# AuburnSounds/gamut

Measured on AMD Instinct MI355X. Metric: Mpixels/sec decoded (batched 1080p JPEG 4:2:0), higher is better.
Workload: dtype int32; 1 GPU; batch 1024 x 1920x1080 baseline JPEG 4:2:0, IDCT + freq-domain chroma upsample + YCbCr->RGBA8, coefficients + max_zag of the q 90 smooth-plus-noise generator; parity_check=not run (bench.py --full checks against the oracle before timing)

## Files before the change

gamut_amd/csrc/jpeg.hip:

```cpp
#include "common.hpp"
#include "jpeg_math.hpp"

namespace gamut {
namespace {

using namespace jpg;

constexpr int TILE_MCUS = 8;
#ifndef JPEG_H2V2_MCUS
#define JPEG_H2V2_MCUS 8
#endif
constexpr int H2V2_MCUS = JPEG_H2V2_MCUS;
constexpr int H2V2_THREADS = 32 * H2V2_MCUS;

struct JpegArgs {
    const int16_t* coeffs; int64_t coeff_stride;
    const uint8_t* max_zag; int64_t zag_stride;
    uint8_t* out; int64_t out_pitch; int64_t out_stride;
    int width, height;
    int mcus_per_row, mcus_per_col;
    int scan_type, out_comps;
    int count;
    const u32* tokens; const u32* strip_tab; const int64_t* tok_offs; const int64_t* strip_offs;
    int nt;
    int flip;
};

constexpr int BLK_STRIDE = 72;
constexpr int T1_INTS = 4 * H2V2_MCUS * BLK_STRIDE;
constexpr int H_INTS  = 2 * H2V2_MCUS * BLK_STRIDE;
constexpr int V_INTS  = 2 * H2V2_MCUS * BLK_STRIDE;
constexpr int LDS_INTS = T1_INTS + H_INTS + V_INTS;

__device__ __forceinline__ constexpr int phys_slot(int m) { constexpr int P[8] = { 0, 2, 1, 3, 6, 4, 7, 5 }; return P[m]; }

__device__ const u32 kMapPacked[2][4] __attribute__((aligned(16))) = {
    { pk16(E1a, E1b), pk16(E1c, E1d), pk16(E3a, E3b), pk16(E3c, E3d) }, { pk16(O0a, O0b), pk16(O0c, O0d), pk16(O2a, O2b), pk16(O2c, O2d) } };
__device__ const i32 kVTable[4][4] __attribute__((aligned(16))) = { { O0a, O0b, O0c, O0d }, { E1a, E1b, E1c, E1d }, { O2a, O2b, O2c, O2d }, { E3a, E3b, E3c, E3d } };
struct __attribute__((packed, aligned(1))) Dwords4u { u32 v[4]; };

__device__ __forceinline__ void wave_sync()
{
    __builtin_amdgcn_fence(__ATOMIC_RELEASE, "wavefront");
    __builtin_amdgcn_wave_barrier();
    __builtin_amdgcn_fence(__ATOMIC_ACQUIRE, "wavefront");
}
#ifndef JPEG_NT_LOADS
#define JPEG_NT_LOADS 1
#endif
__device__ __forceinline__ uint4 load_coeffs16(const int16_t* p)
{
    typedef u32 u32x4n __attribute__((ext_vector_type(4)));
    if (JPEG_NT_LOADS) { const u32x4n v = __builtin_nontemporal_load(reinterpret_cast<const u32x4n*>(p)); return make_uint4(v.x, v.y, v.z, v.w); }
    return *reinterpret_cast<const uint4*>(p);
}

__device__ __forceinline__ void store_px_nt(uint8_t* row_base, u32 voff, u32 px)
{
    asm volatile("global_store_dword %0, %1, %2 nt" :: "v"(voff), "v"(px), "s"(row_base));
}
__device__ __forceinline__ void store_px_plain(uint8_t* row_base, u32 voff, u32 px)
{
    asm volatile("global_store_dword %0, %1, %2" :: "v"(voff), "v"(px), "s"(row_base));
}

#ifndef JPEG_XCD_REMAP
#define JPEG_XCD_REMAP 1
#endif
#ifndef JPEG_STRIPS
#define JPEG_STRIPS 1
#endif
#ifndef JPEG_STRIPS_PACKED
#define JPEG_STRIPS_PACKED 5
#endif
#ifndef JPEG_UNROLL_STRIPS
#define JPEG_UNROLL_STRIPS 0
#endif
#ifndef JPEG_444_MCUS
#define JPEG_444_MCUS 10
#endif
#ifndef JPEG_444_MCUS_RGB8
#define JPEG_444_MCUS_RGB8 8
#endif
constexpr int plain_mcus(int scan_type, int oc = 4) { return scan_type == GAMUT_JPGD_GRAYSCALE ? 32 : scan_type == GAMUT_JPGD_YH1V1 ? (oc == 3 ? JPEG_444_MCUS_RGB8 : JPEG_444_MCUS) : 8; }
constexpr int plain_strips(int scan_type) { return (scan_type == GAMUT_JPGD_GRAYSCALE || scan_type == GAMUT_JPGD_YH1V1) ? 8 : 1; }
constexpr int plain_threads(int scan_type) { return scan_type == GAMUT_JPGD_YH1V1 ? ((JPEG_444_MCUS > JPEG_444_MCUS_RGB8 ? JPEG_444_MCUS : JPEG_444_MCUS_RGB8) * 3 * 8 + 63) / 64 * 64 : 256; }
#ifndef JPEG_ABLATE
#define JPEG_ABLATE 0
#endif

#ifndef JPEG_MIN_WAVES
#define JPEG_MIN_WAVES 0
#endif
template <int OC, bool TOK = false, bool NT = true>
#if JPEG_MIN_WAVES
__global__ __launch_bounds__(H2V2_THREADS, JPEG_MIN_WAVES) void k_jpeg_h2v2(JpegArgs a)
#else
__global__ __launch_bounds__(H2V2_THREADS) void k_jpeg_h2v2(JpegArgs a)
#endif
{
    __shared__ __attribute__((aligned(16))) i32 lds[LDS_INTS];
    i32* const T1 = lds;
    i32* const Hs = T1 + T1_INTS;
    i32* const Vs = Hs + H_INTS;
    i32* const T2 = T1;
    int16_t* const Xs = reinterpret_cast<int16_t*>(Vs);

    constexpr int STRIPS = OC == 4 ? JPEG_STRIPS : JPEG_STRIPS_PACKED;
    const int t = threadIdx.x;
#if JPEG_XCD_REMAP
    const int img = blockIdx.z * 8 + (blockIdx.x & 7), mcu_y = blockIdx.y, tile0 = (blockIdx.x >> 3) * STRIPS;
    if (img >= a.count) return;
#else
    const int img = blockIdx.z, mcu_y = blockIdx.y, tile0 = blockIdx.x * STRIPS;
#endif
    const int n_tiles = (a.mcus_per_row + H2V2_MCUS - 1) / H2V2_MCUS;
    const int16_t* cbase = TOK ? nullptr : a.coeffs + (int64_t)img * a.coeff_stride + ((int64_t)mcu_y * a.mcus_per_row + tile0 * H2V2_MCUS) * (6 * 64);
    uint8_t* obase = a.out + (int64_t)img * a.out_stride + (a.flip ? (int64_t)(a.height - 1 - (mcu_y * 16 + 15)) : (int64_t)(mcu_y * 16)) * a.out_pitch +
                     (int64_t)tile0 * (H2V2_MCUS * 16 * OC);
    const uint8_t* zbase = a.max_zag ? a.max_zag + (int64_t)img * a.zag_stride + ((int64_t)mcu_y * a.mcus_per_row + tile0 * H2V2_MCUS) * 6 : nullptr;

    const int b = t >> 3, r = t & 7, m = b >> 2, q = b & 3;
    const int cbk = t >> 4, k = (t >> 1) & 7, half = t & 1;
    const uint4 mp = *reinterpret_cast<const uint4*>(kMapPacked[half]);
    const int ci = (t >> 2) & 3, cj = t & 3;
    const int pe = ((ci & 1) << 1) | (ci >> 1);
    const int po = 4 + ((((ci & 1) ^ 1) << 1) | (ci >> 1));
    const int4 vc = *reinterpret_cast<const int4*>(kVTable[cj]);
    const i32 sg = (cj & 1) ? -1 : 1;

    const ColourConsts cc = colour_consts();
    const i32 c_round = col_round();
    const int lx = m * 16 + (q & 1) * 8 + r;
    const int ly0 = (q >> 1) * 8;
    const bool all_rows = a.height - mcu_y * 16 >= 16;
    const int rows_here = a.height - mcu_y * 16 - ly0;
    const u32 pitch = (u32)a.out_pitch;
    const u32 voff = (u32)(lx * 4) + (u32)(a.flip ? 8 - ly0 : ly0) * pitch;

    const u32 yoff = (u32)(m * 384 + q * 64 + r * 8), yoff0 = (u32)(q * 64 + r * 8);
    const u32 coff = (u32)((cbk >> 1) * 384 + 256 + (cbk & 1) * 64 + k * 8), coff0 = (u32)(256 + (cbk & 1) * 64 + k * 8);
    auto fetch = [&](int tile, uint4& yv, uint4& cv) {
        const int here = a.mcus_per_row - tile * H2V2_MCUS;
        const int16_t* base = cbase + (int64_t)(tile - tile0) * (H2V2_MCUS * 384);
#if JPEG_ABLATE == 3
        yv = make_uint4(t + tile, t * 3, t * 5, t * 7); cv = make_uint4(t * 11, t, t * 13, t * 17 + tile); (void)here; (void)base;
#else
        yv = load_coeffs16(base + (m < here ? yoff : yoff0));
        cv = load_coeffs16(base + ((cbk >> 1) < here ? coff : coff0));
#endif
    };
    auto fetch_zag = [&](int tile) -> u32 {
        if (!zbase) return 64u;
        const int here = a.mcus_per_row - tile * H2V2_MCUS;
        return m < here ? (u32)zbase[((tile - tile0) * H2V2_MCUS + m) * 6 + q] : 1u;
    };
    auto fetch_tokens = [&](int tile, uint4& yv, uint4& cv) {
        if constexpr (TOK) {
            uint8_t* const ctile = reinterpret_cast<uint8_t*>(Hs);
            __syncthreads();
            static_assert((H_INTS + V_INTS) * 4 >= 64 * 128, "the coefficient tile (any 6-bit block index) fits the H / V area");
            *reinterpret_cast<uint4*>(ctile + t * 16) = make_uint4(0, 0, 0, 0);
            *reinterpret_cast<uint2*>(ctile + H2V2_THREADS * 16 + t * 8) = make_uint2(0, 0);
            const u32* st = a.strip_tab + a.strip_offs[img] + ((int64_t)mcu_y * n_tiles + tile);
            const u32 t0 = st[0], t1 = st[1];
            const u32* tk = a.tokens + a.tok_offs[img];
            __syncthreads();
            for (u32 idx = t0 + (u32)t; idx < t1; idx += H2V2_THREADS) {
                const u32 w = tk[idx];
                *reinterpret_cast<uint16_t*>(ctile + ((w >> 26) << 7) + ((w >> 19) & 126u)) = (uint16_t)w;
            }
            __syncthreads();
            yv = *reinterpret_cast<const uint4*>(ctile + yoff * 2);
            cv = *reinterpret_cast<const uint4*>(ctile + coff * 2);
            __syncthreads();
        }
    };
    uint4 yrow, crow;
    u32 yzag = 64;
    if (!TOK && tile0 < n_tiles) { fetch(tile0, yrow, crow); yzag = fetch_zag(tile0); }

#if JPEG_UNROLL_STRIPS
    #pragma unroll
#else
    #pragma unroll 1
#endif
    for (int s = 0; s < STRIPS; ++s) {
        const int tile = tile0 + s;
        if (tile >= n_tiles) break;
        const int mcu_x0 = tile * H2V2_MCUS;
        const int mcus_here = min(H2V2_MCUS, a.mcus_per_row - mcu_x0);
        const bool mcu_live = m < mcus_here;
        uint8_t* const otile = obase + (size_t)s * (H2V2_MCUS * 16 * OC);
        if constexpr (TOK) { fetch_tokens(tile, yrow, crow); yzag = fetch_zag(tile); }
        uint4 ynext = yrow, cnext = crow;
        u32 znext = yzag;
        if (!TOK && s + 1 < STRIPS && tile + 1 < n_tiles) { fetch(tile + 1, ynext, cnext); znext = fetch_zag(tile + 1); }
        const bool y_sparse = zbase && __builtin_amdgcn_ballot_w64(yzag > 10u) == 0;

#if JPEG_ABLATE == 1
        if constexpr (OC == 4) {
            const u32 v0 = yrow.x ^ yrow.y ^ yrow.z ^ yrow.w ^ crow.x ^ crow.y ^ crow.z ^ crow.w;
            if (mcu_live && mcu_x0 * 16 + lx < a.width && all_rows) {
                #pragma unroll
                for (int i = 0; i < 8; ++i) store_px_nt(otile + (size_t)i * pitch, voff, v0 + i);
            }
            yrow = ynext; crow = cnext; yzag = znext; (void)y_sparse;
            continue;
        }
#endif

        if (y_sparse) {
            i32 tv[8];
            row_pass4_pairs(__builtin_amdgcn_perm(yrow.y, yrow.x, 0x05040100u), __builtin_amdgcn_perm(yrow.y, yrow.x, 0x07060302u), tv);
            if (r < 4) {
                i32* dst = T1 + b * BLK_STRIDE + r * 8;
                *reinterpret_cast<int4*>(dst)     = make_int4(tv[0], tv[1], tv[2], tv[3]);
                *reinterpret_cast<int4*>(dst + 4) = make_int4(tv[4], tv[5], tv[6], tv[7]);
            }
        } else {
            i32 tv[8];
            row_pass_packed(yrow, tv);
            i32* dst = T1 + b * BLK_STRIDE + r * 8;
            *reinterpret_cast<int4*>(dst)     = make_int4(tv[0], tv[1], tv[2], tv[3]);
            *reinterpret_cast<int4*>(dst + 4) = make_int4(tv[4], tv[5], tv[6], tv[7]);
        }
        {
            i32 hv[4];
            const u32 w0 = half ? crow.y : crow.x, w1 = half ? crow.w : crow.z;
            const u32 p13 = __builtin_amdgcn_perm(crow.y, crow.x, 0x07060302u), p57 = __builtin_amdgcn_perm(crow.w, crow.z, 0x07060302u);
            hv[0] = (i32)(short)(w0 & 0xFFFF);
            hv[1] = (i32)(short)(w1 & 0xFFFF);
            hv[2] = dot2(p13, mp.x, dot2(p57, mp.y, 512)) >> 10;
            hv[3] = dot2(p13, mp.z, dot2(p57, mp.w, 512)) >> 10;
            *reinterpret_cast<int4*>(Hs + cbk * BLK_STRIDE + k * 8 + half * 4) = make_int4(hv[0], hv[1], hv[2], hv[3]);
        }
        wave_sync();

        i32 ys[8];
        {
            const i32* src = T1 + b * BLK_STRIDE + r;
            i32 t0;
            if (y_sparse) {
                t0 = src[0];
                col_pass4_direct(t0, src[8], src[16], src[24], ys, c_round);
            } else {
                i32 tv[8];
                #pragma unroll
                for (int i = 0; i < 8; ++i) tv[i] = src[i * 8];
                col_pass<8>(tv, ys);
                t0 = tv[0];
            }
            if (zbase && __builtin_amdgcn_ballot_w64(yzag <= 2u) != 0) {
                const bool y_col1 = mcu_live && yzag <= 2u;
                const i32 v = col1_sample(t0);
                #pragma unroll
                for (int i = 0; i < 8; ++i) ys[i] = y_col1 ? v : ys[i];
            }
        }
        {
            const i32* he = Hs + cbk * BLK_STRIDE + pe;
            const i32* ho = Hs + cbk * BLK_STRIDE + po;
            const i32 pass_e = he[cj * 16], pass_o = ho[cj * 16];
            const i32 sum_e = mad24_1(vc.w, he[56], mad24_1(vc.z, he[40], mad24_1(vc.y, he[24], mad24_1(vc.x, he[8], 512)))) >> 10;
            const i32 sum_o = mad24_1(vc.w, ho[56], mad24_1(vc.z, ho[40], mad24_1(vc.y, ho[24], mad24_1(vc.x, ho[8], 512)))) >> 10;
            const i32 pa = wadd(pass_e, sum_e), pc = wadd(pass_o, sum_o);
            const i32 pu = wsub(pass_e, sum_e), pv = wsub(pass_o, sum_o);
            int16_t* dst = Xs + cbk * 64 + cj * 4 + pe;
            dst[0]  = (int16_t)wadd(pa, pc);
            dst[16] = (int16_t)wsub(pa, pc);
            dst[32] = (int16_t)mad24_1(wadd(pu, pv), sg, 0);
            dst[48] = (int16_t)mad24_1(wsub(pu, pv), sg, 0);
        }
        wave_sync();

        {
            const int mm = t >> 5, comp = (t >> 4) & 1, qq = (t >> 2) & 3, j = t & 3;
            const uint2 xp = *reinterpret_cast<const uint2*>(Xs + (mm * 2 + comp) * 64 + qq * 16 + j * 4);
            i32 tv[8];
            row_pass4_pairs(xp.x, xp.y, tv);
            i32* dst = T2 + (mm * 4 + qq) * BLK_STRIDE + (comp * 4 + j) * 8;
            *reinterpret_cast<int4*>(dst)     = make_int4(tv[0], tv[1], tv[2], tv[3]);
            *reinterpret_cast<int4*>(dst + 4) = make_int4(tv[4], tv[5], tv[6], tv[7]);
        }
        wave_sync();

        {
            i32 cbs[8], crs[8];
            const i32* src = T2 + b * BLK_STRIDE + r;
            col_pass4_direct(src[0], src[8], src[16], src[24], cbs, c_round);
            col_pass4_direct(src[32], src[40], src[48], src[56], crs, c_round);

            const bool px_live = mcu_live && mcu_x0 * 16 + lx < a.width;
            if constexpr (OC == 4) {
                auto store_px = [](uint8_t* row_base, u32 vo, u32 px) { if constexpr (NT) store_px_nt(row_base, vo, px); else store_px_plain(row_base, vo, px); };
                if (px_live) {
                    if (JPEG_ABLATE == 2) {
                        u32 acc = 0;
                        #pragma unroll
                        for (int i = 0; i < 8; ++i) acc += ycc_to_rgba(ys[i], cbs[i], crs[i], cc.kr, cc.kb, cc.kg);
                        if (acc == 0x12345679u) store_px_nt(otile, voff, acc);
                    } else
                    if (all_rows) {
                        #pragma unroll
                        for (int i = 0; i < 8; ++i) store_px(otile + (size_t)(a.flip ? 7 - i : i) * pitch, voff, ycc_to_rgba(ys[i], cbs[i], crs[i], cc.kr, cc.kb, cc.kg));
                    } else {
                        #pragma unroll
                        for (int i = 0; i < 8; ++i)
                            if (i < rows_here) store_px(otile + (size_t)(a.flip ? 7 - i : i) * pitch, voff, ycc_to_rgba(ys[i], cbs[i], crs[i], cc.kr, cc.kb, cc.kg));
                    }
                }
            } else {
                static_assert(OC == 3 || OC == 1, "output components");
                constexpr int BPR = 16 * H2V2_MCUS * OC;
                uint8_t* stage = reinterpret_cast<uint8_t*>(Hs);
                const int j = lx & 3;
                __syncthreads();
                #pragma unroll
                for (int i = 0; i < 8; ++i) {
                    const u32 px = ycc_to_rgba(ys[i], cbs[i], crs[i], cc.kr, cc.kb, cc.kg);
                    if constexpr (OC == 3) {
                        const u32 sel = j == 0 ? 0x04020100u : j == 1 ? 0x05040201u : 0x06050402u;
                        const u32 nx = (u32)__builtin_amdgcn_mov_dpp((int)px, 0xF9, 0xF, 0xF, true);
                        const u32 dw = __builtin_amdgcn_perm(nx, px, sel);
                        if (j < 3) *reinterpret_cast<u32*>(stage + (ly0 + i) * BPR + lx * 3 + j) = dw;
                    } else {
                        u32 v = rgb_to_luma(px) << (8 * j);
                        v |= (u32)__builtin_amdgcn_mov_dpp((int)v, 0xB1, 0xF, 0xF, true);
                        v |= (u32)__builtin_amdgcn_mov_dpp((int)v, 0x4E, 0xF, 0xF, true);
                        if (j == 0) *reinterpret_cast<u32*>(stage + (ly0 + i) * BPR + lx) = v;
                    }
                }
                __syncthreads();
                const int row_bytes = min(mcus_here * 16, a.width - mcu_x0 * 16) * OC;
                const int live_rows = min(16, a.height - mcu_y * 16);
                constexpr int CPR = BPR / 16;
                for (int c = t; c < 16 * CPR; c += H2V2_THREADS) {
                    const int row = c / CPR, off = (c - row * CPR) * 16;
                    if (row >= live_rows || off >= row_bytes) continue;
                    const uint4 v = *reinterpret_cast<const uint4*>(stage + row * BPR + off);
                    uint8_t* o = otile + (u32)(a.flip ? 15 - row : row) * pitch + (u32)off;
                    if (off + 16 <= row_bytes) {
                        if (a.nt) {
                            typedef u32 u32x4p __attribute__((ext_vector_type(4), aligned(4)));
                            __builtin_nontemporal_store(u32x4p{ v.x, v.y, v.z, v.w }, reinterpret_cast<u32x4p*>(o));
                        } else {
                            Dwords4u d; d.v[0] = v.x; d.v[1] = v.y; d.v[2] = v.z; d.v[3] = v.w;
                            *reinterpret_cast<Dwords4u*>(o) = d;
                        }
                    } else {
                        const u32 w[4] = { v.x, v.y, v.z, v.w };
                        for (int kk = 0; kk < row_bytes - off; ++kk) o[kk] = (uint8_t)(w[kk >> 2] >> ((kk & 3) * 8));
                    }
                }
                __syncthreads();
            }
        }
        wave_sync();
        yrow = ynext; crow = cnext; yzag = znext;
    }
}

struct __attribute__((packed, aligned(4))) Dwords4 { u32 v[4]; };
struct __attribute__((packed, aligned(1))) Dwords3 { u32 v[3]; };
struct __attribute__((packed, aligned(1))) Dword1 { u32 v; };

template <int ST, int OC, bool NT = true>
__global__ __launch_bounds__(plain_threads(ST)) void k_jpeg_plain(JpegArgs a)
{
    constexpr int NTHR = plain_threads(ST);
    static_assert(ST == GAMUT_JPGD_GRAYSCALE || ST == GAMUT_JPGD_YH1V1 || ST == GAMUT_JPGD_YH2V1 || ST == GAMUT_JPGD_YH1V2, "sampling mode");
    constexpr int BPM  = ST == GAMUT_JPGD_GRAYSCALE ? 1 : ST == GAMUT_JPGD_YH1V1 ? 3 : 4;
    constexpr int MH   = ST == GAMUT_JPGD_YH1V2 ? 16 : 8;
    constexpr int MCUS = plain_mcus(ST, OC);
    constexpr int NBLK = MCUS * BPM;
    static_assert(NBLK * 8 <= NTHR, "a thread per block row");
    constexpr int MW   = ST == GAMUT_JPGD_YH2V1 ? 16 : 8;
    constexpr int SW   = MCUS * MW;
    __shared__ __attribute__((aligned(16))) i32 T1[NBLK * BLK_STRIDE];
    __shared__ __attribute__((aligned(16))) uint8_t S[NBLK * 64];

    const int t = threadIdx.x;
    const int img = blockIdx.z * 8 + (blockIdx.x & 7), mcu_y = blockIdx.y, bx = blockIdx.x >> 3;
    if (img >= a.count) return;
    constexpr int PLAIN_STRIPS = plain_strips(ST);
    for (int strip = 0; strip < PLAIN_STRIPS; ++strip) {
    const int mcu_x0 = (bx * PLAIN_STRIPS + strip) * MCUS;
    if (mcu_x0 >= a.mcus_per_row) break;
    const int64_t blk0 = ((int64_t)mcu_y * a.mcus_per_row + mcu_x0) * BPM;
    const int16_t* cbase = a.coeffs + (int64_t)img * a.coeff_stride + blk0 * 64;
    const int mcus_here = min(MCUS, a.mcus_per_row - mcu_x0);
    const int b = t >> 3, r = t & 7;
    const bool blk_live = b < mcus_here * BPM;

    if (t < NBLK * 8) {
        uint4 row = make_uint4(0, 0, 0, 0);
        if (blk_live) row = load_coeffs16(cbase + (u32)(t * 8));
        i32 tv[8];
        row_pass_packed(row, tv);
        i32* dst = T1 + b * BLK_STRIDE + r * 8;
        *reinterpret_cast<int4*>(dst)     = make_int4(tv[0], tv[1], tv[2], tv[3]);
        *reinterpret_cast<int4*>(dst + 4) = make_int4(tv[4], tv[5], tv[6], tv[7]);
    }
    wave_sync();
    if (t < NBLK * 8) {
        i32 tv[8], sm[8];
        const i32* src = T1 + b * BLK_STRIDE + r;
        #pragma unroll
        for (int i = 0; i < 8; ++i) tv[i] = src[i * 8];
        col_pass<8>(tv, sm);
        if (a.max_zag) {
            bool col1 = false;
            if (blk_live) col1 = a.max_zag[(int64_t)img * a.zag_stride + blk0 + b] <= 2;
            const i32 v = col1_sample(tv[0]);
            #pragma unroll
            for (int i = 0; i < 8; ++i) sm[i] = col1 ? v : sm[i];
        }
        #pragma unroll
        for (int i = 0; i < 8; ++i) S[b * 64 + i * 8 + r] = (uint8_t)sm[i];
    }
    __syncthreads();

    uint8_t* obase = a.out + (int64_t)img * a.out_stride + (int64_t)(mcu_y * MH) * a.out_pitch + (int64_t)mcu_x0 * (MW * OC);
    const int rows_here = min(MH, a.height - mcu_y * MH);
    const int px_here = min(mcus_here * MW, a.width - mcu_x0 * MW);
    constexpr int GPR = SW / 4;
    for (int g = t; g < GPR * MH; g += NTHR) {
        const int y = g / GPR, x0 = (g - y * GPR) * 4;
        if (y >= rows_here || x0 >= px_here) continue;
        const int m = x0 / MW, xin = x0 - m * MW;
        u32 ys, px[4];
        if constexpr (ST == GAMUT_JPGD_GRAYSCALE) {
            ys = *reinterpret_cast<const u32*>(S + m * 64 + y * 8 + xin);
        } else if constexpr (ST == GAMUT_JPGD_YH1V1) {
            const uint8_t* sp = S + m * 192 + y * 8 + xin;
            ys = *reinterpret_cast<const u32*>(sp);
            const u32 cbs = *reinterpret_cast<const u32*>(sp + 64), crs = *reinterpret_cast<const u32*>(sp + 128);
            #pragma unroll
            for (int j = 0; j < 4; ++j) px[j] = ycc_to_rgba((ys >> (8 * j)) & 255, (cbs >> (8 * j)) & 255, (crs >> (8 * j)) & 255);
        } else if constexpr (ST == GAMUT_JPGD_YH1V2) {
            const uint8_t* mp = S + m * 256;
            ys = *reinterpret_cast<const u32*>(mp + (y >> 3) * 64 + (y & 7) * 8 + xin);
// ... 348 lines not shown
        i32 yv;
        if (st == GAMUT_JPGD_GRAYSCALE) {
            yv = s[ly * 8 + xin]; rgba = 0;
        } else if (st == GAMUT_JPGD_YH1V1) {
            const int o = ly * 8 + xin;
            yv = s[o]; rgba = ycc_to_rgba(yv, s[64 + o], s[128 + o]);
        } else if (st == GAMUT_JPGD_YH2V1) {
            yv = s[(xin >> 3) * 64 + ly * 8 + (xin & 7)];
            const int co = 2 * 64 + ly * 8 + (xin >> 1);
            rgba = ycc_to_rgba(yv, s[co], s[co + 64]);
        } else if (st == GAMUT_JPGD_YH1V2) {
            yv = s[(ly >> 3) * 64 + (ly & 7) * 8 + xin];
            const int co = 2 * 64 + (ly >> 1) * 8 + xin;
            rgba = ycc_to_rgba(yv, s[co], s[co + 64]);
        } else {
            const int o = ((ly >> 3) * 2 + (xin >> 3)) * 64 + (ly & 7) * 8 + (xin & 7);
            yv = s[o]; rgba = ycc_to_rgba(yv, s[4 * 64 + o], s[8 * 64 + o]);
        }
        uint8_t* o = obase + (int64_t)gy * a.out_pitch + (int64_t)gx * a.out_comps;
        if (st == GAMUT_JPGD_GRAYSCALE) {
            o[0] = (uint8_t)yv;
            if (a.out_comps >= 3) { o[1] = o[2] = (uint8_t)yv; if (a.out_comps == 4) o[3] = 255; }
        } else if (a.out_comps == 4) {
            o[0] = (uint8_t)rgba; o[1] = (uint8_t)(rgba >> 8); o[2] = (uint8_t)(rgba >> 16); o[3] = 255;
        } else if (a.out_comps == 3) {
            o[0] = (uint8_t)rgba; o[1] = (uint8_t)(rgba >> 8); o[2] = (uint8_t)(rgba >> 16);
        } else {
            o[0] = (uint8_t)rgb_to_luma(rgba);
        }
    }
}

}

int jpeg_reconstruct_launch(const int16_t* coeffs, int64_t coeff_stride,
                            const uint8_t* max_zag, int64_t zag_stride,
                            uint8_t* out, int64_t out_pitch, int64_t out_stride,
                            int width, int height, int scan_type, int out_comps,
                            int count, hipStream_t stream)
{
    if (width < 1 || height < 1 || width > 16384 || height > 16384)
        return set_error(GAMUT_HIP_ERR_INVALID_ARG, "jpeg_reconstruct: bad image size %dx%d", width, height);
    if (scan_type < GAMUT_JPGD_GRAYSCALE || scan_type > GAMUT_JPGD_YH2V2)
        return set_error(GAMUT_HIP_ERR_INVALID_ARG, "jpeg_reconstruct: bad scan type %d", scan_type);
    if (out_comps != 1 && out_comps != 3 && out_comps != 4)
        return set_error(GAMUT_HIP_ERR_INVALID_ARG, "jpeg_reconstruct: out_comps must be 1, 3 or 4");
    if (count < 0) return set_error(GAMUT_HIP_ERR_INVALID_ARG, "jpeg_reconstruct: negative count");
    if (count == 0) return GAMUT_HIP_OK;
    if (!coeffs || !out) return set_error(GAMUT_HIP_ERR_INVALID_ARG, "jpeg_reconstruct: null pointer");
    if (((uintptr_t)coeffs & 15) || (count > 1 && (coeff_stride & 7)))
        return set_error(GAMUT_HIP_ERR_INVALID_ARG, "jpeg_reconstruct: coefficient buffers must be 16-byte aligned");

    JpegArgs a{};
    a.coeffs = coeffs; a.coeff_stride = coeff_stride; a.max_zag = max_zag; a.zag_stride = zag_stride;
    a.out = out; a.out_pitch = out_pitch; a.out_stride = out_stride;
    a.width = width; a.height = height; a.scan_type = scan_type; a.out_comps = out_comps;
    const int mcu_w = (scan_type == GAMUT_JPGD_YH2V1 || scan_type == GAMUT_JPGD_YH2V2) ? 16 : 8;
    const int mcu_h = (scan_type == GAMUT_JPGD_YH1V2 || scan_type == GAMUT_JPGD_YH2V2) ? 16 : 8;
    a.mcus_per_row = (width + mcu_w - 1) / mcu_w;
    a.mcus_per_col = (height + mcu_h - 1) / mcu_h;
    const int tiles = (a.mcus_per_row + TILE_MCUS - 1) / TILE_MCUS;

    for (int i0 = 0; i0 < count; i0 += 65535) {
        const int n = count - i0 < 65535 ? count - i0 : 65535;
        JpegArgs c = a;
        c.count = n;
        c.coeffs += (int64_t)i0 * coeff_stride; c.out += (int64_t)i0 * out_stride;
        if (c.max_zag) c.max_zag += (int64_t)i0 * zag_stride;
        const dim3 grid(tiles, a.mcus_per_col, n);
        const int64_t apitch = out_pitch < 0 ? -out_pitch : out_pitch;
        const bool tuned = apitch > 0 && apitch < (1 << 27) &&
                           (out_comps != 4 || (((uintptr_t)out & 3) == 0 && (apitch & 3) == 0 && (out_stride & 3) == 0));
        if (tuned && out_pitch < 0 && scan_type == GAMUT_JPGD_YH2V2) { c.flip = 1; c.out_pitch = apitch; c.out += (int64_t)(height - 1) * out_pitch; }
        const bool on_lines = (((uintptr_t)out | (uintptr_t)apitch | (uintptr_t)(count > 1 ? (out_stride < 0 ? -out_stride : out_stride) : 0)) & 127u) == 0;
        c.nt = on_lines ? 1 : 0;
        const char* const cols_env = getenv("GAMUT_HIP_JPEG_COLS");
        const bool cols_tuned = !(cols_env && !strcmp(cols_env, "plain"));
        const int ps = plain_strips(scan_type);
        const int pm = plain_mcus(scan_type, out_comps);
        const dim3 grid32(8u * (unsigned)(((a.mcus_per_row + 31) / 32 + ps - 1) / ps), a.mcus_per_col, (n + 7) / 8);
        const dim3 grid_plain(8u * (unsigned)(((a.mcus_per_row + pm - 1) / pm + ps - 1) / ps), a.mcus_per_col, (n + 7) / 8);
        const int strips420 = out_comps == 4 ? JPEG_STRIPS : JPEG_STRIPS_PACKED;
        const unsigned groups420 = (unsigned)(((a.mcus_per_row + H2V2_MCUS - 1) / H2V2_MCUS + strips420 - 1) / strips420);
#if JPEG_XCD_REMAP
        const dim3 grid420(8u * groups420, a.mcus_per_col, (n + 7) / 8);
#else
        const dim3 grid420(groups420, a.mcus_per_col, n);
#endif
#define GAMUT_JPEG_PLAIN(ST, G) do { \
            if (out_comps == 4)      hipLaunchKernelGGL((k_jpeg_plain<ST, 4>), G, dim3(plain_threads(ST)), 0, stream, c);       \
            else if (out_comps == 3) { if (on_lines) hipLaunchKernelGGL((k_jpeg_plain<ST, 3>), G, dim3(plain_threads(ST)), 0, stream, c); else hipLaunchKernelGGL((k_jpeg_plain<ST, 3, false>), G, dim3(plain_threads(ST)), 0, stream, c); } \
            else                     { if (on_lines) hipLaunchKernelGGL((k_jpeg_plain<ST, 1>), G, dim3(plain_threads(ST)), 0, stream, c); else hipLaunchKernelGGL((k_jpeg_plain<ST, 1, false>), G, dim3(plain_threads(ST)), 0, stream, c); } } while (0)
        if (!tuned)                                   hipLaunchKernelGGL(k_jpeg_generic, grid, dim3(256), 0, stream, c);
        else if (scan_type == GAMUT_JPGD_GRAYSCALE)   GAMUT_JPEG_PLAIN(GAMUT_JPGD_GRAYSCALE, grid32);
        else if ((scan_type == GAMUT_JPGD_YH1V1 || scan_type == GAMUT_JPGD_GRAYSCALE) && cols_tuned) {
            const int waste32 = (32 - a.mcus_per_row % 32) % 32, waste24 = (24 - a.mcus_per_row % 24) % 24;
            const bool m24 = waste24 * 32 < waste32 * 24;
            const dim3 g(8u * (unsigned)(((a.mcus_per_row + (m24 ? 23 : 31)) / (m24 ? 24 : 32) + 1) / 2), a.mcus_per_col, (n + 7) / 8);
#define GAMUT_JPEG_COLS(ST, OC) do { if (m24) { if (on_lines) hipLaunchKernelGGL((k_jpeg_cols<ST, OC, 24>), g, dim3(192), 0, stream, c); else hipLaunchKernelGGL((k_jpeg_cols<ST, OC, 24, false>), g, dim3(192), 0, stream, c); } \
                                     else     { if (on_lines) hipLaunchKernelGGL((k_jpeg_cols<ST, OC, 32>), g, dim3(256), 0, stream, c); else hipLaunchKernelGGL((k_jpeg_cols<ST, OC, 32, false>), g, dim3(256), 0, stream, c); } } while (0)
            if (scan_type == GAMUT_JPGD_YH1V1) { if (out_comps == 4) GAMUT_JPEG_COLS(GAMUT_JPGD_YH1V1, 4); else if (out_comps == 3) GAMUT_JPEG_COLS(GAMUT_JPGD_YH1V1, 3); else GAMUT_JPEG_COLS(GAMUT_JPGD_YH1V1, 1); }
            else                               { if (out_comps == 4) GAMUT_JPEG_COLS(GAMUT_JPGD_GRAYSCALE, 4); else if (out_comps == 3) GAMUT_JPEG_COLS(GAMUT_JPGD_GRAYSCALE, 3); else GAMUT_JPEG_COLS(GAMUT_JPGD_GRAYSCALE, 1); }
#undef GAMUT_JPEG_COLS
        }
        else if (scan_type == GAMUT_JPGD_YH1V1)       GAMUT_JPEG_PLAIN(GAMUT_JPGD_YH1V1, grid_plain);
        else if ((scan_type == GAMUT_JPGD_YH2V1 || scan_type == GAMUT_JPGD_YH1V2) && cols_tuned) {
            const int waste32 = (32 - a.mcus_per_row % 32) % 32, waste24 = (24 - a.mcus_per_row % 24) % 24;
            const bool m24 = waste24 * 32 < waste32 * 24;
            const dim3 g(8u * (unsigned)(((a.mcus_per_row + (m24 ? 23 : 31)) / (m24 ? 24 : 32) + 1) / 2), a.mcus_per_col, (n + 7) / 8);
#define GAMUT_JPEG_COLS4(ST, OC) do { if (m24) { if (on_lines) hipLaunchKernelGGL((k_jpeg_cols4<ST, OC, 24>), g, dim3(192), 0, stream, c); else hipLaunchKernelGGL((k_jpeg_cols4<ST, OC, 24, false>), g, dim3(192), 0, stream, c); } \
                                      else     { if (on_lines) hipLaunchKernelGGL((k_jpeg_cols4<ST, OC, 32>), g, dim3(256), 0, stream, c); else hipLaunchKernelGGL((k_jpeg_cols4<ST, OC, 32, false>), g, dim3(256), 0, stream, c); } } while (0)
            if (scan_type == GAMUT_JPGD_YH2V1) { if (out_comps == 4) GAMUT_JPEG_COLS4(GAMUT_JPGD_YH2V1, 4); else if (out_comps == 3) GAMUT_JPEG_COLS4(GAMUT_JPGD_YH2V1, 3); else GAMUT_JPEG_COLS4(GAMUT_JPGD_YH2V1, 1); }
            else                               { if (out_comps == 4) GAMUT_JPEG_COLS4(GAMUT_JPGD_YH1V2, 4); else if (out_comps == 3) GAMUT_JPEG_COLS4(GAMUT_JPGD_YH1V2, 3); else GAMUT_JPEG_COLS4(GAMUT_JPGD_YH1V2, 1); }
#undef GAMUT_JPEG_COLS4
        }
        else if (scan_type == GAMUT_JPGD_YH2V1)       GAMUT_JPEG_PLAIN(GAMUT_JPGD_YH2V1, grid_plain);
        else if (scan_type == GAMUT_JPGD_YH1V2)       GAMUT_JPEG_PLAIN(GAMUT_JPGD_YH1V2, grid_plain);
        else if (out_comps == 4 && on_lines) hipLaunchKernelGGL(k_jpeg_h2v2<4>, grid420, dim3(H2V2_THREADS), 0, stream, c);
        else if (out_comps == 4) hipLaunchKernelGGL((k_jpeg_h2v2<4, false, false>), grid420, dim3(H2V2_THREADS), 0, stream, c);
        else if (out_comps == 3) hipLaunchKernelGGL(k_jpeg_h2v2<3>, grid420, dim3(H2V2_THREADS), 0, stream, c);
        else                     hipLaunchKernelGGL(k_jpeg_h2v2<1>, grid420, dim3(H2V2_THREADS), 0, stream, c);
#undef GAMUT_JPEG_PLAIN
        if (int rc = launch_status("jpeg_reconstruct")) return rc;
    }
    return GAMUT_HIP_OK;
}

int jpeg_reconstruct_tokens_launch(const uint32_t* tokens, const uint32_t* strip_tab, const int64_t* tok_offs, const int64_t* strip_offs,
                                   const uint8_t* max_zag, int64_t zag_stride, uint8_t* out, int64_t out_pitch, int64_t out_stride,
                                   int width, int height, int out_comps, int count, hipStream_t stream)
{
    if (width < 1 || height < 1 || width > 16384 || height > 16384 || count < 0 || (out_comps != 1 && out_comps != 3 && out_comps != 4) || !max_zag)
        return set_error(GAMUT_HIP_ERR_INVALID_ARG, "jpeg_reconstruct_tokens: bad arguments");
    if (count == 0) return GAMUT_HIP_OK;
    const int64_t apitch = out_pitch < 0 ? -out_pitch : out_pitch;
    if (apitch <= 0 || apitch >= (1 << 27) || (out_comps == 4 && ((((uintptr_t)out & 3) != 0) || (apitch & 3) || (out_stride & 3))))
        return set_error(GAMUT_HIP_ERR_INVALID_ARG, "jpeg_reconstruct_tokens: output rows must be dword-aligned for rgba8");
    JpegArgs a{};
    a.tokens = tokens; a.strip_tab = strip_tab; a.max_zag = max_zag; a.zag_stride = zag_stride;
    a.out = out; a.out_pitch = apitch; a.out_stride = out_stride;
    a.width = width; a.height = height; a.scan_type = GAMUT_JPGD_YH2V2; a.out_comps = out_comps;
    a.mcus_per_row = (width + 15) / 16; a.mcus_per_col = (height + 15) / 16;
    if (out_pitch < 0) { a.flip = 1; a.out += (int64_t)(height - 1) * out_pitch; }
    for (int i0 = 0; i0 < count; i0 += 65528) {
        const int n = count - i0 < 65528 ? count - i0 : 65528;
        JpegArgs c = a;
        c.count = n; c.out += (int64_t)i0 * out_stride; c.max_zag += (int64_t)i0 * zag_stride; c.tok_offs = tok_offs + i0; c.strip_offs = strip_offs + i0;
        const int strips420 = out_comps == 4 ? JPEG_STRIPS : JPEG_STRIPS_PACKED;
        const unsigned groups420 = (unsigned)(((a.mcus_per_row + H2V2_MCUS - 1) / H2V2_MCUS + strips420 - 1) / strips420);
#if JPEG_XCD_REMAP
        const dim3 grid420(8u * groups420, a.mcus_per_col, (n + 7) / 8);
#else
        const dim3 grid420(groups420, a.mcus_per_col, n);
#endif
        const bool on_lines = (((uintptr_t)out | (uintptr_t)apitch | (uintptr_t)(count > 1 ? (out_stride < 0 ? -out_stride : out_stride) : 0)) & 127u) == 0;
        c.nt = on_lines ? 1 : 0;
        if (out_comps == 4 && on_lines) hipLaunchKernelGGL((k_jpeg_h2v2<4, true>), grid420, dim3(H2V2_THREADS), 0, stream, c);
        else if (out_comps == 4) hipLaunchKernelGGL((k_jpeg_h2v2<4, true, false>), grid420, dim3(H2V2_THREADS), 0, stream, c);
        else if (out_comps == 3) hipLaunchKernelGGL((k_jpeg_h2v2<3, true>), grid420, dim3(H2V2_THREADS), 0, stream, c);
        else                     hipLaunchKernelGGL((k_jpeg_h2v2<1, true>), grid420, dim3(H2V2_THREADS), 0, stream, c);
        if (int rc = launch_status("jpeg_reconstruct_tokens")) return rc;
    }
    return GAMUT_HIP_OK;
}

}
```

Before: 813,900 Mpx/s.

## Split packed RGB/gray 4:2:0 path into its own software-pipelined kernel

Moves the OC==3/1 4:2:0 reconstruction into a separate kernel that uses buffer-resource loads, forces arguments into scalar registers, and overlaps the next strip's row pass with the current strip's staged store. It also adds a col-1 shortcut for very sparse Y blocks. The grid choice (XCD remap vs plain) becomes a runtime flag selected when the batch has fewer than 8 images. The benchmarked RGBA8 path only gains a PLAIN template variant and loses the OC branches, so it should be mostly unchanged for batch 1024.

```diff
diff --git a/gamut_amd/csrc/jpeg.hip b/gamut_amd/csrc/jpeg.hip
--- a/gamut_amd/csrc/jpeg.hip
+++ b/gamut_amd/csrc/jpeg.hip
@@ -21,6 +21,7 @@
     int mcus_per_row, mcus_per_col;
     int scan_type, out_comps;
     int count;
+    int plain_grid;
     const u32* tokens; const u32* strip_tab; const int64_t* tok_offs; const int64_t* strip_offs;
     int nt;
     int flip;
@@ -92,7 +93,7 @@
 #ifndef JPEG_MIN_WAVES
 #define JPEG_MIN_WAVES 0
 #endif
-template <int OC, bool TOK = false, bool NT = true>
+template <int OC, bool TOK = false, bool NT = true, bool PLAIN = false>
 #if JPEG_MIN_WAVES
 __global__ __launch_bounds__(H2V2_THREADS, JPEG_MIN_WAVES) void k_jpeg_h2v2(JpegArgs a)
 #else
@@ -106,14 +107,12 @@
     i32* const T2 = T1;
     int16_t* const Xs = reinterpret_cast<int16_t*>(Vs);
 
-    constexpr int STRIPS = OC == 4 ? JPEG_STRIPS : JPEG_STRIPS_PACKED;
+    static_assert(OC == 4, "rgba8");
+    constexpr int STRIPS = JPEG_STRIPS;
     const int t = threadIdx.x;
-#if JPEG_XCD_REMAP
-    const int img = blockIdx.z * 8 + (blockIdx.x & 7), mcu_y = blockIdx.y, tile0 = (blockIdx.x >> 3) * STRIPS;
+    const int img = PLAIN ? (int)blockIdx.z : (int)(blockIdx.z * 8 + (blockIdx.x & 7));
+    const int mcu_y = blockIdx.y, tile0 = (int)(PLAIN ? blockIdx.x : blockIdx.x >> 3) * STRIPS;
     if (img >= a.count) return;
-#else
-    const int img = blockIdx.z, mcu_y = blockIdx.y, tile0 = blockIdx.x * STRIPS;
-#endif
     const int n_tiles = (a.mcus_per_row + H2V2_MCUS - 1) / H2V2_MCUS;
     const int16_t* cbase = TOK ? nullptr : a.coeffs + (int64_t)img * a.coeff_stride + ((int64_t)mcu_y * a.mcus_per_row + tile0 * H2V2_MCUS) * (6 * 64);
     uint8_t* obase = a.out + (int64_t)img * a.out_stride + (a.flip ? (int64_t)(a.height - 1 - (mcu_y * 16 + 15)) : (int64_t)(mcu_y * 16)) * a.out_pitch +
@@ -199,7 +198,7 @@
         const bool y_sparse = zbase && __builtin_amdgcn_ballot_w64(yzag > 10u) == 0;
 
 #if JPEG_ABLATE == 1
-        if constexpr (OC == 4) {
+        {
             const u32 v0 = yrow.x ^ yrow.y ^ yrow.z ^ yrow.w ^ crow.x ^ crow.y ^ crow.z ^ crow.w;
             if (mcu_live && mcu_x0 * 16 + lx < a.width && all_rows) {
                 #pragma unroll
@@ -292,7 +291,7 @@
             col_pass4_direct(src[32], src[40], src[48], src[56], crs, c_round);
 
             const bool px_live = mcu_live && mcu_x0 * 16 + lx < a.width;
-            if constexpr (OC == 4) {
+            {
                 auto store_px = [](uint8_t* row_base, u32 vo, u32 px) { if constexpr (NT) store_px_nt(row_base, vo, px); else store_px_plain(row_base, vo, px); };
                 if (px_live) {
                     if (JPEG_ABLATE == 2) {
@@ -310,11 +309,211 @@
                             if (i < rows_here) store_px(otile + (size_t)(a.flip ? 7 - i : i) * pitch, voff, ycc_to_rgba(ys[i], cbs[i], crs[i], cc.kr, cc.kb, cc.kg));
                     }
                 }
+            }
+        }
+        wave_sync();
+        yrow = ynext; crow = cnext; yzag = znext;
+    }
+}
+
+template <int OC, bool TOK = false>
+__global__ __launch_bounds__(H2V2_THREADS) void k_jpeg_h2v2_packed(JpegArgs a)
+{
+    __shared__ __attribute__((aligned(16))) i32 lds[LDS_INTS];
+    i32* const T1 = lds;
+    i32* const Hs = T1 + T1_INTS;
+    i32* const Vs = Hs + H_INTS;
+    i32* const T2 = T1;
+    int16_t* const Xs = reinterpret_cast<int16_t*>(Vs);
+
+    static_assert(OC == 3 || OC == 1, "output components");
+    constexpr int STRIPS = JPEG_STRIPS_PACKED;
+    const int t = threadIdx.x;
+    if constexpr (TOK)
+        asm volatile("" :: "s"(a.tokens), "s"(a.strip_tab), "s"(a.tok_offs), "s"(a.strip_offs), "s"(a.max_zag), "s"(a.zag_stride), "s"(a.out), "s"(a.out_pitch), "s"(a.out_stride),
+                           "s"(a.width), "s"(a.height), "s"(a.mcus_per_row), "s"(a.count), "s"(a.nt), "s"(a.flip), "s"(a.plain_grid));
+    else
+        asm volatile("" :: "s"(a.coeffs), "s"(a.coeff_stride), "s"(a.max_zag), "s"(a.zag_stride), "s"(a.out), "s"(a.out_pitch), "s"(a.out_stride),
+                           "s"(a.width), "s"(a.height), "s"(a.mcus_per_row), "s"(a.count), "s"(a.nt), "s"(a.flip), "s"(a.plain_grid));
+    const int img = a.plain_grid ? (int)blockIdx.z : (int)(blockIdx.z * 8 + (blockIdx.x & 7));
+    const int mcu_y = blockIdx.y, tile0 = (int)(a.plain_grid ? blockIdx.x : blockIdx.x >> 3) * STRIPS;
+    if (img >= a.count) return;
+    const int n_tiles = (a.mcus_per_row + H2V2_MCUS - 1) / H2V2_MCUS;
+    const int n_run = min(STRIPS, n_tiles - tile0);
+    if (n_run < 1) return;
+    const int last_tile = n_tiles - 1;
+    const int here_last = a.mcus_per_row - last_tile * H2V2_MCUS;
+    const int16_t* const cbase = TOK ? nullptr : a.coeffs + (int64_t)img * a.coeff_stride + ((int64_t)mcu_y * a.mcus_per_row + tile0 * H2V2_MCUS) * (6 * 64);
+    uint8_t* const obase = a.out + (int64_t)img * a.out_stride + (a.flip ? (int64_t)(a.height - 1 - (mcu_y * 16 + 15)) : (int64_t)(mcu_y * 16)) * a.out_pitch +
+                           (int64_t)tile0 * (H2V2_MCUS * 16 * OC);
+    const uint8_t* const zbase = a.max_zag ? a.max_zag + (int64_t)img * a.zag_stride + ((int64_t)mcu_y * a.mcus_per_row + tile0 * H2V2_MCUS) * 6 : nullptr;
+
+    const int b = t >> 3, r = t & 7, m = b >> 2, q = b & 3;
+    const int cbk = t >> 4, k = (t >> 1) & 7, half = t & 1;
+    const uint4 mp = *reinterpret_cast<const uint4*>(kMapPacked[half]);
+    const int ci = (t >> 2) & 3, cj = t & 3;
+    const int pe = ((ci & 1) << 1) | (ci >> 1);
+    const int po = 4 + ((((ci & 1) ^ 1) << 1) | (ci >> 1));
+    const int4 vc = *reinterpret_cast<const int4*>(kVTable[cj]);
+    const i32 sg = (cj & 1) ? -1 : 1;
+
+    const ColourConsts cc = colour_consts();
+    const i32 c_round = col_round();
+    const int lx = m * 16 + (q & 1) * 8 + r;
+    const int ly0 = (q >> 1) * 8;
+    const u32 pitch = (u32)a.out_pitch;
+    const bool live_last = m < here_last;
+
+    const u32 yoff = (u32)(m * 384 + q * 64 + r * 8);
+    const u32 coff = (u32)(m * 384 + 256 + (cbk & 1) * 64 + k * 8);
+    const u32 zoff = (u32)(m * 6 + q);
+    uint4 yrow, crow;
+    u32 yzag = 64;
+    const int row_mcus_left = a.mcus_per_row - tile0 * H2V2_MCUS;
+    const __amdgpu_buffer_rsrc_t crsrc = __builtin_amdgcn_make_buffer_rsrc(const_cast<int16_t*>(cbase), 0, TOK ? 0 : row_mcus_left * 768, 0x00020000);
+    const __amdgpu_buffer_rsrc_t zrsrc = __builtin_amdgcn_make_buffer_rsrc(const_cast<uint8_t*>(zbase), 0, zbase ? row_mcus_left * 6 : 0, 0x00020000);
+    auto fetch = [&](int tile) {
+        const u32 back = (tile == last_tile && !live_last) ? (u32)(m * 6) : 0u;
+        const int strip = tile - tile0;
+        typedef u32 u32x4b __attribute__((ext_vector_type(4)));
+        const u32x4b yv = __builtin_amdgcn_raw_buffer_load_b128(crsrc, (int)((yoff - back * 64u) * 2u), strip * (H2V2_MCUS * 768), JPEG_NT_LOADS ? 2 : 0);
+        const u32x4b cv = __builtin_amdgcn_raw_buffer_load_b128(crsrc, (int)((coff - back * 64u) * 2u), strip * (H2V2_MCUS * 768), JPEG_NT_LOADS ? 2 : 0);
+        yrow = make_uint4(yv.x, yv.y, yv.z, yv.w); crow = make_uint4(cv.x, cv.y, cv.z, cv.w);
+        if (zbase) yzag = (u32)__builtin_amdgcn_raw_buffer_load_b8(zrsrc, (int)(zoff - back), strip * (H2V2_MCUS * 6), 0);
+    };
+    auto fetch_tokens = [&](int tile) {
+        if constexpr (TOK) {
+            uint8_t* const ctile = reinterpret_cast<uint8_t*>(Hs);
+            __syncthreads();
+            static_assert((H_INTS + V_INTS) * 4 >= 64 * 128, "the coefficient tile (any 6-bit block index) fits the H / V area");
+            *reinterpret_cast<uint4*>(ctile + t * 16) = make_uint4(0, 0, 0, 0);
+            *reinterpret_cast<uint2*>(ctile + H2V2_THREADS * 16 + t * 8) = make_uint2(0, 0);
+            const u32* st = a.strip_tab + a.strip_offs[img] + ((int64_t)mcu_y * n_tiles + tile);
+            const u32 t0 = st[0], t1 = st[1];
+            const u32* tk = a.tokens + a.tok_offs[img];
+            __syncthreads();
+            for (u32 idx = t0 + (u32)t; idx < t1; idx += H2V2_THREADS) {
+                const u32 w = tk[idx];
+                *reinterpret_cast<uint16_t*>(ctile + ((w >> 26) << 7) + ((w >> 19) & 126u)) = (uint16_t)w;
+            }
+            __syncthreads();
+            yrow = *reinterpret_cast<const uint4*>(ctile + yoff * 2);
+            crow = *reinterpret_cast<const uint4*>(ctile + coff * 2);
+            __syncthreads();
+            const u32 back = (tile == last_tile && !live_last) ? (u32)(m * 6) : 0u;
+            yzag = (u32)__builtin_amdgcn_raw_buffer_load_b8(zrsrc, (int)(zoff - back), (tile - tile0) * (H2V2_MCUS * 6), 0);
+        }
+    };
+    bool y_sparse = false;
+    bool y_col1 = false, any_col1 = false;
+    auto pass1 = [&]() {
+        y_sparse = zbase && __builtin_amdgcn_ballot_w64(yzag > 10u) == 0;
+        y_col1 = yzag <= 2u;
+        any_col1 = zbase && __builtin_amdgcn_ballot_w64(y_col1) != 0;
+        if (y_sparse) {
+            i32 tv[8];
+            row_pass4_pairs(__builtin_amdgcn_perm(yrow.y, yrow.x, 0x05040100u), __builtin_amdgcn_perm(yrow.y, yrow.x, 0x07060302u), tv);
+            if (r < 4) {
+                i32* dst = T1 + b * BLK_STRIDE + r * 8;
+                *reinterpret_cast<int4*>(dst)     = make_int4(tv[0], tv[1], tv[2], tv[3]);
+                *reinterpret_cast<int4*>(dst + 4) = make_int4(tv[4], tv[5], tv[6], tv[7]);
+            }
+        } else {
+            i32 tv[8];
+            row_pass_packed(yrow, tv);
+            i32* dst = T1 + b * BLK_STRIDE + r * 8;
+            *reinterpret_cast<int4*>(dst)     = make_int4(tv[0], tv[1], tv[2], tv[3]);
+            *reinterpret_cast<int4*>(dst + 4) = make_int4(tv[4], tv[5], tv[6], tv[7]);
+        }
+        {
+            i32 hv[4];
+            const u32 w0 = half ? crow.y : crow.x, w1 = half ? crow.w : crow.z;
+            const u32 p13 = __builtin_amdgcn_perm(crow.y, crow.x, 0x07060302u), p57 = __builtin_amdgcn_perm(crow.w, crow.z, 0x07060302u);
+            hv[0] = (i32)(short)(w0 & 0xFFFF);
+            hv[1] = (i32)(short)(w1 & 0xFFFF);
+            hv[2] = dot2(p13, mp.x, dot2(p57, mp.y, 512)) >> 10;
+            hv[3] = dot2(p13, mp.z, dot2(p57, mp.w, 512)) >> 10;
+            *reinterpret_cast<int4*>(Hs + cbk * BLK_STRIDE + k * 8 + half * 4) = make_int4(hv[0], hv[1], hv[2], hv[3]);
+        }
+    };
+    if constexpr (TOK) fetch_tokens(tile0); else fetch(tile0);
+    pass1();
+
+#if JPEG_UNROLL_STRIPS
+    #pragma unroll
+#else
+    #pragma unroll 1
+#endif
+    for (int s = 0; s < n_run; ++s) {
+        const int tile = tile0 + s;
+        const bool more = s + 1 < n_run;
+        uint8_t* const otile = obase + (size_t)s * (H2V2_MCUS * 16 * OC);
+        auto next_pass1 = [&]() {
+            wave_sync();
+            if (more) { if constexpr (TOK) fetch_tokens(tile + 1); pass1(); }
+        };
+        if (!TOK && more) fetch(tile + 1);
+        wave_sync();
+
+        i32 ys[8];
+        {
+            const i32* src = T1 + b * BLK_STRIDE + r;
+            i32 t0;
+            if (y_sparse) {
+                t0 = src[0];
+                col_pass4_direct(t0, src[8], src[16], src[24], ys, c_round);
             } else {
-                static_assert(OC == 3 || OC == 1, "output components");
+                i32 tv[8];
+                #pragma unroll
+                for (int i = 0; i < 8; ++i) tv[i] = src[i * 8];
+                col_pass<8>(tv, ys);
+                t0 = tv[0];
+            }
+            if (any_col1) {
+                const i32 v = col1_sample(t0);
+                #pragma unroll
+                for (int i = 0; i < 8; ++i) ys[i] = y_col1 ? v : ys[i];
+            }
+        }
+        {
+            const i32* he = Hs + cbk * BLK_STRIDE + pe;
+            const i32* ho = Hs + cbk * BLK_STRIDE + po;
+            const i32 pass_e = he[cj * 16], pass_o = ho[cj * 16];
+            const i32 sum_e = mad24_1(vc.w, he[56], mad24_1(vc.z, he[40], mad24_1(vc.y, he[24], mad24_1(vc.x, he[8], 512)))) >> 10;
+            const i32 sum_o = mad24_1(vc.w, ho[56], mad24_1(vc.z, ho[40], mad24_1(vc.y, ho[24], mad24_1(vc.x, ho[8], 512)))) >> 10;
+            const i32 pa = wadd(pass_e, sum_e), pc = wadd(pass_o, sum_o);
+            const i32 pu = wsub(pass_e, sum_e), pv = wsub(pass_o, sum_o);
+            int16_t* dst = Xs + cbk * 64 + cj * 4 + pe;
+            dst[0]  = (int16_t)wadd(pa, pc);
+            dst[16] = (int16_t)wsub(pa, pc);
+            dst[32] = (int16_t)mad24_1(wadd(pu, pv), sg, 0);
+            dst[48] = (int16_t)mad24_1(wsub(pu, pv), sg, 0);
+        }
+        wave_sync();
+
+        {
+            const int mm = t >> 5, comp = (t >> 4) & 1, qq = (t >> 2) & 3, j = t & 3;
+            const uint2 xp = *reinterpret_cast<const uint2*>(Xs + (mm * 2 + comp) * 64 + qq * 16 + j * 4);
+            i32 tv[8];
+            row_pass4_pairs(xp.x, xp.y, tv);
+            i32* dst = T2 + (mm * 4 + qq) * BLK_STRIDE + (comp * 4 + j) * 8;
+            *reinterpret_cast<int4*>(dst)     = make_int4(tv[0], tv[1], tv[2], tv[3]);
+            *reinterpret_cast<int4*>(dst + 4) = make_int4(tv[4], tv[5], tv[6], tv[7]);
+        }
+        wave_sync();
+
+        {
+            i32 cbs[8], crs[8];
+            const i32* src = T2 + b * BLK_STRIDE + r;
+            col_pass4_direct(src[0], src[8], src[16], src[24], cbs, c_round);
+            col_pass4_direct(src[32], src[40], src[48], src[56], crs, c_round);
+
+            {
                 constexpr int BPR = 16 * H2V2_MCUS * OC;
                 uint8_t* stage = reinterpret_cast<uint8_t*>(Hs);
                 const int j = lx & 3;
+                const int mcu_x0 = tile * H2V2_MCUS;
+                const int mcus_here = min(H2V2_MCUS, a.mcus_per_row - mcu_x0);
                 __syncthreads();
                 #pragma unroll
                 for (int i = 0; i < 8; ++i) {
@@ -354,10 +553,9 @@
                     }
                 }
                 __syncthreads();
-            }
-        }
-        wave_sync();
-        yrow = ynext; crow = cnext; yzag = znext;
+                next_pass1();
+            }
+        }
     }
 }
 
@@ -872,11 +1070,8 @@
         const dim3 grid_plain(8u * (unsigned)(((a.mcus_per_row + pm - 1) / pm + ps - 1) / ps), a.mcus_per_col, (n + 7) / 8);
         const int strips420 = out_comps == 4 ? JPEG_STRIPS : JPEG_STRIPS_PACKED;
         const unsigned groups420 = (unsigned)(((a.mcus_per_row + H2V2_MCUS - 1) / H2V2_MCUS + strips420 - 1) / strips420);
-#if JPEG_XCD_REMAP
-        const dim3 grid420(8u * groups420, a.mcus_per_col, (n + 7) / 8);
-#else
-        const dim3 grid420(groups420, a.mcus_per_col, n);
-#endif
+        c.plain_grid = (!JPEG_XCD_REMAP || n < 8) ? 1 : 0;
+        const dim3 grid420 = c.plain_grid ? dim3(groups420, a.mcus_per_col, n) : dim3(8u * groups420, a.mcus_per_col, (n + 7) / 8);
 #define GAMUT_JPEG_PLAIN(ST, G) do { \
             if (out_comps == 4)      hipLaunchKernelGGL((k_jpeg_plain<ST, 4>), G, dim3(plain_threads(ST)), 0, stream, c);       \
             else if (out_comps == 3) { if (on_lines) hipLaunchKernelGGL((k_jpeg_plain<ST, 3>), G, dim3(plain_threads(ST)), 0, stream, c); else hipLaunchKernelGGL((k_jpeg_plain<ST, 3, false>), G, dim3(plain_threads(ST)), 0, stream, c); } \
@@ -906,10 +1101,12 @@
         }
         else if (scan_type == GAMUT_JPGD_YH2V1)       GAMUT_JPEG_PLAIN(GAMUT_JPGD_YH2V1, grid_plain);
         else if (scan_type == GAMUT_JPGD_YH1V2)       GAMUT_JPEG_PLAIN(GAMUT_JPGD_YH1V2, grid_plain);
+        else if (out_comps == 4 && on_lines && c.plain_grid) hipLaunchKernelGGL((k_jpeg_h2v2<4, false, true, true>), grid420, dim3(H2V2_THREADS), 0, stream, c);
+        else if (out_comps == 4 && c.plain_grid) hipLaunchKernelGGL((k_jpeg_h2v2<4, false, false, true>), grid420, dim3(H2V2_THREADS), 0, stream, c);
         else if (out_comps == 4 && on_lines) hipLaunchKernelGGL(k_jpeg_h2v2<4>, grid420, dim3(H2V2_THREADS), 0, stream, c);
         else if (out_comps == 4) hipLaunchKernelGGL((k_jpeg_h2v2<4, false, false>), grid420, dim3(H2V2_THREADS), 0, stream, c);
-        else if (out_comps == 3) hipLaunchKernelGGL(k_jpeg_h2v2<3>, grid420, dim3(H2V2_THREADS), 0, stream, c);
-        else                     hipLaunchKernelGGL(k_jpeg_h2v2<1>, grid420, dim3(H2V2_THREADS), 0, stream, c);
+        else if (out_comps == 3) hipLaunchKernelGGL(k_jpeg_h2v2_packed<3>, grid420, dim3(H2V2_THREADS), 0, stream, c);
+        else                     hipLaunchKernelGGL(k_jpeg_h2v2_packed<1>, grid420, dim3(H2V2_THREADS), 0, stream, c);
 #undef GAMUT_JPEG_PLAIN
         if (int rc = launch_status("jpeg_reconstruct")) return rc;
     }
@@ -938,17 +1135,16 @@
         c.count = n; c.out += (int64_t)i0 * out_stride; c.max_zag += (int64_t)i0 * zag_stride; c.tok_offs = tok_offs + i0; c.strip_offs = strip_offs + i0;
         const int strips420 = out_comps == 4 ? JPEG_STRIPS : JPEG_STRIPS_PACKED;
         const unsigned groups420 = (unsigned)(((a.mcus_per_row + H2V2_MCUS - 1) / H2V2_MCUS + strips420 - 1) / strips420);
-#if JPEG_XCD_REMAP
-        const dim3 grid420(8u * groups420, a.mcus_per_col, (n + 7) / 8);
-#else
-        const dim3 grid420(groups420, a.mcus_per_col, n);
-#endif
+        c.plain_grid = (!JPEG_XCD_REMAP || n < 8) ? 1 : 0;
+        const dim3 grid420 = c.plain_grid ? dim3(groups420, a.mcus_per_col, n) : dim3(8u * groups420, a.mcus_per_col, (n + 7) / 8);
         const bool on_lines = (((uintptr_t)out | (uintptr_t)apitch | (uintptr_t)(count > 1 ? (out_stride < 0 ? -out_stride : out_stride) : 0)) & 127u) == 0;
         c.nt = on_lines ? 1 : 0;
-        if (out_comps == 4 && on_lines) hipLaunchKernelGGL((k_jpeg_h2v2<4, true>), grid420, dim3(H2V2_THREADS), 0, stream, c);
+        if (out_comps == 4 && on_lines && c.plain_grid) hipLaunchKernelGGL((k_jpeg_h2v2<4, true, true, true>), grid420, dim3(H2V2_THREADS), 0, stream, c);
+        else if (out_comps == 4 && c.plain_grid) hipLaunchKernelGGL((k_jpeg_h2v2<4, true, false, true>), grid420, dim3(H2V2_THREADS), 0, stream, c);
+        else if (out_comps == 4 && on_lines) hipLaunchKernelGGL((k_jpeg_h2v2<4, true>), grid420, dim3(H2V2_THREADS), 0, stream, c);
         else if (out_comps == 4) hipLaunchKernelGGL((k_jpeg_h2v2<4, true, false>), grid420, dim3(H2V2_THREADS), 0, stream, c);
-        else if (out_comps == 3) hipLaunchKernelGGL((k_jpeg_h2v2<3, true>), grid420, dim3(H2V2_THREADS), 0, stream, c);
-        else                     hipLaunchKernelGGL((k_jpeg_h2v2<1, true>), grid420, dim3(H2V2_THREADS), 0, stream, c);
+        else if (out_comps == 3) hipLaunchKernelGGL((k_jpeg_h2v2_packed<3, true>), grid420, dim3(H2V2_THREADS), 0, stream, c);
+        else                     hipLaunchKernelGGL((k_jpeg_h2v2_packed<1, true>), grid420, dim3(H2V2_THREADS), 0, stream, c);
         if (int rc = launch_status("jpeg_reconstruct_tokens")) return rc;
     }
     return GAMUT_HIP_OK;
```

New measurement: 814,800 Mpx/s, median of 2. No clear change (+0.1%).
